# wseaton/gpu-pruner

Hardware: NVIDIA H100
Metric: dcgm_samples_reduced_per_sec (higher is better)
Workload: dtype f32

## Files before the change

### gpu-pruner_b200/csrc/gpr_api.cu

```cuda
#include "../../include/gpr.h"

#include <cuda_runtime.h>
#include <dlfcn.h>
#include <nccl.h>
#include <nvtx3/nvToolsExt.h>

#include <algorithm>
#include <atomic>
#include <chrono>
#include <cmath>
#include <cstdarg>
#include <cstdio>
#include <cstdlib>
#include <cstring>
#include <mutex>
#include <new>
#include <thread>
#include <vector>

#include "gpr_kernels.cuh"
#include "gpr_groups.cuh"
#include "gpr_ring.cuh"
#include "gpr_synth.cuh"
#include "gpr_text_kernels.cuh"

namespace {

using gpr::kLdgUnroll;
using gpr::kLdgWarps;
using gpr::kTmaSmemBudget;
constexpr int kSlots = 256;
constexpr int kMaxChunkEvents = 64;
constexpr int kExchangeDepth = 4;

std::mutex g_err_mu;
char g_create_err[512] = "";

struct NcclApi {
  void* handle = nullptr;
  ncclResult_t (*GetUniqueId)(ncclUniqueId*) = nullptr;
  ncclResult_t (*CommInitRank)(ncclComm_t*, int, ncclUniqueId, int) = nullptr;
  ncclResult_t (*CommDestroy)(ncclComm_t) = nullptr;
  ncclResult_t (*AllGather)(const void*, void*, size_t, ncclDataType_t, ncclComm_t,
                            cudaStream_t) = nullptr;
  const char* (*GetErrorString)(ncclResult_t) = nullptr;
  bool ok = false;
};
NcclApi g_nccl;
std::mutex g_nccl_mu;

bool load_nccl(char* err, size_t n) {
  std::lock_guard<std::mutex> lk(g_nccl_mu);
  if (g_nccl.ok) return true;
  const char* names[] = {"libnccl.so.2", "libnccl.so"};
  for (const char* nm : names) {
    g_nccl.handle = dlopen(nm, RTLD_NOW | RTLD_GLOBAL);
    if (g_nccl.handle) break;
  }
  if (!g_nccl.handle) {
    snprintf(err, n, "NCCL not loadable: %s", dlerror());
    return false;
  }
#define GPR_SYM(field, name)                                              \
  g_nccl.field = reinterpret_cast<decltype(g_nccl.field)>(dlsym(g_nccl.handle, name)); \
  if (!g_nccl.field) {                                                    \
    snprintf(err, n, "NCCL symbol %s missing", name);                     \
    return false;                                                         \
  }
  GPR_SYM(GetUniqueId, "ncclGetUniqueId")
  GPR_SYM(CommInitRank, "ncclCommInitRank")
  GPR_SYM(CommDestroy, "ncclCommDestroy")
  GPR_SYM(AllGather, "ncclAllGather")
  GPR_SYM(GetErrorString, "ncclGetErrorString")
#undef GPR_SYM
  g_nccl.ok = true;
  return true;
}

struct Pending {
  gpr_result* res;
  int slot;
};

}

struct gpr_ctx {
  int device = 0;
  cudaStream_t stream = nullptr;
  bool own_stream = false;
  cudaStream_t copy_stream = nullptr;
  cudaEvent_t ev_k0 = nullptr, ev_k1 = nullptr, ev_t0 = nullptr, ev_t1 = nullptr;
  cudaEvent_t ev_join = nullptr;
  cudaEvent_t ev_chunk[kMaxChunkEvents] = {};
  int sm_count = 0;
  size_t l2_bytes = 0, hbm_bytes = 0;
  int cc_major = 0, cc_minor = 0;
  char name[64] = "";
  int variant = GPR_KERNEL_AUTO;
  int ldg_ctas_per_sm = 2;
  int tma_depth_max = 3;
  int tma_warps = 16;
  int tma_chunk_bytes = 8192;
  size_t chunk_bytes = 32u << 20;
  int parse_ctas_per_sm = 6;

  uint32_t max_pods = 0, max_gpus = 0, max_samples = 0;
  bool cap_power = false;
  float* d_util_stage = nullptr;
  float* d_power_stage = nullptr;
  uint8_t* d_elig_stage = nullptr;
  int64_t* d_created_stage = nullptr;
  size_t gate_cap = 0;

  uint32_t* d_masks[2] = {nullptr, nullptr};
  size_t masks_cap[2] = {0, 0};
  bool masks_dirty = false;
  unsigned int* d_tickets = nullptr;
  unsigned long long* d_acc = nullptr;
  unsigned long long* d_done = nullptr;
  unsigned long long uses[2] = {0, 0};
  unsigned parity = 0;
  bool pdl_enabled = true;
  bool last_was_reduce = false;
  uint32_t* d_bits = nullptr;
  size_t bits_cap = 0;
  uint32_t* d_gather = nullptr;
  size_t gather_cap = 0;
  float* d_smax = nullptr;
  size_t smax_cap = 0;
  uint32_t* d_grouped = nullptr;
  size_t grouped_cap = 0;
  uint32_t* d_gpods = nullptr;
  size_t gpods_cap = 0;
  float* d_gmax = nullptr;
  size_t gmax_cap = 0;
  uint32_t* d_gtable = nullptr;
  size_t gtable_cap = 0;
  uint32_t* d_islots = nullptr;
  size_t islots_cap = 0;
  unsigned int* h_gerr = nullptr;
  unsigned long long* h_counts = nullptr;
  unsigned long long* h_mark = nullptr;
  unsigned int* h_err = nullptr;
  std::vector<Pending> pending;
  std::vector<uint64_t> stamps;
  std::vector<uint64_t> phase_stamps;
  unsigned long long rdv_seq = 0;

  void* d_flush = nullptr;
  size_t flush_bytes = 0;

  float* d_res_util = nullptr;
  float* d_res_power = nullptr;
  uint32_t res_P = 0, res_G = 0, res_T = 0, res_head = 0;
  float* d_idx_util = nullptr;
  float* d_idx_power = nullptr;
  uint32_t idx_ld = 0;
  bool idx_stale = false;
  float* d_cols = nullptr;
  size_t cols_cap = 0;

  uint8_t* d_text[3] = {nullptr, nullptr, nullptr};
  size_t text_cap[3] = {0, 0, 0};
  uint64_t text_n[3] = {0, 0, 0};
  uint64_t* d_marks = nullptr;
  size_t marks_cap = 0;
  unsigned long long* d_mark_counts = nullptr;
  gpr::text::Span* d_spans = nullptr;
  size_t spans_cap = 0;
  float* d_tplane[2] = {nullptr, nullptr};
  size_t tplane_cap[2] = {0, 0};
  static constexpr int kUpThreads = 16, kUpSlots = 2;
  static constexpr size_t kPinnedChunk = 16u << 20;
  static constexpr int kMarkBlocks = 64;
  static constexpr uint32_t kMarkCap = 16384;
  size_t up_chunk = 2u << 20;
  size_t up_slot_bytes = 0;
  unsigned char* h_up_ring = nullptr;
  uint32_t* h_mark_blocks = nullptr;
  uint32_t* d_mark_blocks = nullptr;
  cudaStream_t up_stream[kUpThreads] = {};
  cudaEvent_t up_event[kUpThreads][kUpSlots] = {};
  cudaEvent_t mark_event[kMarkBlocks] = {};
  int up_threads = 8;
  struct ScanPipe* pipe = nullptr;

  ncclComm_t comm = nullptr;
  int rank = 0, world = 1;
  unsigned char* p2p_block = nullptr;
  unsigned char* p2p_peer[gpr::kMaxPeers] = {};
  size_t p2p_gather_off[kExchangeDepth] = {};
  size_t p2p_ll_off[kExchangeDepth] = {};
  bool exchange_ll = true;
  bool exchange_late = false;
  int fold_threads = 256;
  uint32_t p2p_stride = 0;
  bool p2p_ready = false;
  int exchange_debug = 0;
  unsigned int poll_ns = 4000;
  unsigned long long p2p_step = 0;

  uint64_t launches = 0;
  char err[512] = "";
};

void scan_pipe_abort(gpr_ctx* ctx);

namespace {

int fail(gpr_ctx* c, int code, const char* fmt, ...) {
  char buf[512];
  va_list ap;
  va_start(ap, fmt);
  vsnprintf(buf, sizeof buf, fmt, ap);
  va_end(ap);
  if (c) {
    snprintf(c->err, sizeof c->err, "%s", buf);
  } else {
    std::lock_guard<std::mutex> lk(g_err_mu);
    snprintf(g_create_err, sizeof g_create_err, "%s", buf);
  }
  return code;
}

#define CU(call)                                                                          \
  do {                                                                                    \
    cudaError_t e_ = (call);                                                              \
    if (e_ != cudaSuccess)                                                                \
      return fail(ctx, e_ == cudaErrorMemoryAllocation ? GPR_E_NOMEM : GPR_E_CUDA,        \
                  "%s: %s (%s:%d)", #call, cudaGetErrorString(e_), __FILE__, __LINE__);   \
  } while (0)

#define NC(call)                                                                          \
  do {                                                                                    \
    ncclResult_t r_ = (call);                                                             \
    if (r_ != ncclSuccess)                                                                \
      return fail(ctx, GPR_E_NCCL, "%s: %s", #call, g_nccl.GetErrorString(r_));           \
  } while (0)

template <typename T>
int grow(gpr_ctx* ctx, T** p, size_t* cap, size_t need) {
  if (need <= *cap) return GPR_OK;
  if (*p) {
    CU(cudaStreamSynchronize(ctx->stream));
    CU(cudaFree(*p));
    *p = nullptr;
    *cap = 0;
  }
  size_t want = need + need / 4 + 64;
  CU(cudaMalloc(reinterpret_cast<void**>(p), want * sizeof(T)));
  *cap = want;
  return GPR_OK;
}

int env_int(const char* name, int dflt) {
  const char* v = getenv(name);
  return (v && *v) ? atoi(v) : dflt;
}

bool aligned16(const void* p) { return (reinterpret_cast<uintptr_t>(p) & 15u) == 0; }

float threshold_f32(double thr) { return gpr::text::threshold_up(thr); }

bool power_truthy(double thr) { return thr != 0.0 && !std::isnan(thr); }

gpr::LaunchKnobs launch_knobs(const gpr_ctx* ctx) {
  gpr::LaunchKnobs k;
  k.sm_count = ctx->sm_count;
  k.variant = ctx->variant;
  k.ldg_ctas_per_sm = ctx->ldg_ctas_per_sm;
  k.tma_warps = ctx->tma_warps;
  k.tma_chunk_bytes = ctx->tma_chunk_bytes;
  k.tma_depth_max = ctx->tma_depth_max;
  k.fold_threads = ctx->fold_threads;
  return k;
}

template <typename Kernel, typename... Args>
cudaError_t launch_ex(Kernel k, uint32_t grid, uint32_t block, size_t smem, cudaStream_t st, bool pdl,
                      Args... args) {
  cudaLaunchConfig_t cfg = {};
  cfg.gridDim = dim3(grid), cfg.blockDim = dim3(block), cfg.dynamicSmemBytes = smem, cfg.stream = st;
  cudaLaunchAttribute attr[1];
  attr[0].id = cudaLaunchAttributeProgrammaticStreamSerialization;
  attr[0].val.programmaticStreamSerializationAllowed = 1;
  cfg.attrs = attr;
  cfg.numAttrs = pdl ? 1 : 0;
  return cudaLaunchKernelEx(&cfg, k, args...);
}

template <int NW, bool kGroups>
cudaError_t launch_tma(gpr_ctx* ctx, const gpr::ReduceParams& rp, const gpr::ReducePlan& plan, bool pdl) {
  return launch_ex(gpr::k_reduce_tma<NW, kGroups>, plan.grid, plan.block, plan.smem, ctx->stream, pdl, rp, plan.L);
}

template <bool kGroups>
int launch_reduce_as(gpr_ctx* ctx, gpr::ReduceParams& rp, bool tma_ok, bool pdl) {
  if (rp.total_rows == 0) return GPR_OK;
  const gpr::ReducePlan plan = gpr::plan_reduce(launch_knobs(ctx), rp.T, rp.total_rows, tma_ok, rp.util_u8 != 0);
  cudaError_t e;
  if (plan.kernel == gpr::kReduceU8) {
    e = launch_ex(gpr::k_reduce_u8<kLdgWarps, gpr::kU8Unroll, kGroups>, plan.grid, plan.block, 0, ctx->stream, pdl, rp);
  } else if (plan.kernel == gpr::kReduceTma) {
    const int nw = ctx->tma_warps;
    if (nw == 4) e = launch_tma<4, kGroups>(ctx, rp, plan, pdl);
    else if (nw == 16) e = launch_tma<16, kGroups>(ctx, rp, plan, pdl);
    else if (nw == 32) e = launch_tma<32, kGroups>(ctx, rp, plan, pdl);
    else e = launch_tma<8, kGroups>(ctx, rp, plan, pdl);
  } else {
    e = launch_ex(gpr::k_reduce_ldg<kLdgWarps, kLdgUnroll, kGroups>, plan.grid, plan.block, 0, ctx->stream, pdl, rp);
  }
  ctx->launches++;
  CU(e);
  CU(cudaGetLastError());
  return GPR_OK;
}
int launch_reduce(gpr_ctx* ctx, gpr::ReduceParams& rp, bool tma_ok, bool pdl) {
  return rp.grouped ? launch_reduce_as<true>(ctx, rp, tma_ok, pdl) : launch_reduce_as<false>(ctx, rp, tma_ok, pdl);
}

int copy_rows_h2d(gpr_ctx* ctx, void* dst, const void* src, size_t n_rows, uint32_t T,
                  uint64_t ld, size_t esize, cudaStream_t s) {
  if (n_rows == 0) return GPR_OK;
  if (ld == T) {
    CU(cudaMemcpyAsync(dst, src, n_rows * (size_t)T * esize, cudaMemcpyHostToDevice, s));
  } else {
    CU(cudaMemcpy2DAsync(dst, (size_t)T * esize, src, (size_t)ld * esize, (size_t)T * esize, n_rows,
                         cudaMemcpyHostToDevice, s));
  }
  return GPR_OK;
}

struct NvtxRange {
  explicit NvtxRange(const char* name) { nvtxRangePushA(name); }
  ~NvtxRange() { nvtxRangePop(); }
};

int decide_impl(gpr_ctx* ctx, const gpr_window* win, gpr_result* res, bool resident, bool async) {
  if (!ctx) return GPR_E_INVALID;
  NvtxRange nvtx_range(resident ? "gpr_decide_resident" : "gpr_decide");
  if (!win || !res) return fail(ctx, GPR_E_INVALID, "window/result is NULL");
  const size_t win_v1 = offsetof(gpr_window, groups), res_v1 = offsetof(gpr_result, idle_slots);
  if ((win->struct_size != sizeof(gpr_window) && win->struct_size != win_v1) ||
      (res->struct_size != sizeof(gpr_result) && res->struct_size != res_v1))
    return fail(ctx, GPR_E_INVALID, "struct_size mismatch (window %u/%zu or %zu, result %u/%zu or %zu)",
                win->struct_size, sizeof(gpr_window), win_v1, res->struct_size, sizeof(gpr_result), res_v1);
  const uint32_t* const groups = win->struct_size == sizeof(gpr_window) ? win->groups : nullptr;
  uint32_t* const idle_slots = res->struct_size == sizeof(gpr_result) ? res->idle_slots : nullptr;
  CU(cudaSetDevice(ctx->device));

  uint32_t P = win->n_pods, G = win->n_gpus, T = win->n_samples;
  uint64_t ld = win->row_stride ? win->row_stride : T;
  const float* util = win->util;
  const float* power = win->power;
  int in_kind = win->mem_kind;
  const bool u8 = !resident && win->util_format == GPR_FMT_U8B;
  if (!resident && win->util_format != GPR_FMT_F32 && win->util_format != GPR_FMT_U8B)
    return fail(ctx, GPR_E_INVALID, "bad util_format %u", win->util_format);
  if (resident) {
    if (!ctx->d_res_util) return fail(ctx, GPR_E_STATE, "no resident window (gpr_resident_init)");
    P = ctx->res_P, G = ctx->res_G, T = ctx->res_T, ld = T;
    util = ctx->d_res_util;
    power = ctx->d_res_power;
    if (ctx->d_idx_util) {
      if (ctx->idx_stale)
        return fail(ctx, GPR_E_STATE, "the block index is stale: gpr_text_parse(GPR_TEXT_RESIDENT) merged samples "
                    "into the ring; call gpr_resident_reindex before gpr_decide_resident");
      T = ctx->idx_ld, ld = ctx->idx_ld;
      util = ctx->d_idx_util;
      power = ctx->d_idx_power;
    }
  }
  if (in_kind != GPR_MEM_HOST && in_kind != GPR_MEM_DEVICE)
    return fail(ctx, GPR_E_INVALID, "bad mem_kind %d", in_kind);
  if (res->out_mem_kind != GPR_MEM_HOST && res->out_mem_kind != GPR_MEM_DEVICE)
    return fail(ctx, GPR_E_INVALID, "bad out_mem_kind %d", res->out_mem_kind);
  if (G == 0 || T == 0) return fail(ctx, GPR_E_INVALID, "n_gpus and n_samples must be > 0");
  if (G > 256) return fail(ctx, GPR_E_UNSUPPORTED, "n_gpus %u > 256 series slots per pod is not supported", G);
  const uint32_t MW = (G + 31u) / 32u;
  if (ld < T) return fail(ctx, GPR_E_INVALID, "row_stride %llu < n_samples %u",
                          (unsigned long long)ld, T);
  if (P > 0 && !util) return fail(ctx, GPR_E_INVALID, "util is NULL");
  if (!res->decision_bits && P > 0) return fail(ctx, GPR_E_INVALID, "decision_bits is NULL");
  const uint64_t S64 = (uint64_t)P * G;
  if (S64 > 0x7fffffffull) return fail(ctx, GPR_E_INVALID, "too many series (%llu)",
                                       (unsigned long long)S64);
  const uint32_t S = (uint32_t)S64;
  const uint32_t W = (P + 31u) / 32u;
  const bool use_power = power != nullptr && power_truthy(win->power_threshold);
  const bool host_in = !resident && in_kind == GPR_MEM_HOST;
  const bool gates_host = in_kind == GPR_MEM_HOST;
  const bool host_out = res->out_mem_kind == GPR_MEM_HOST;
  const bool fused = ctx->p2p_ready && ctx->world > 1;
  const bool comm = (ctx->comm != nullptr || fused) && ctx->world > 1;
  if (fused && 2u * W > ctx->p2p_stride)
    return fail(ctx, GPR_E_CAPACITY, "n_pods %u exceeds the p2p exchange capacity (%u pods per rank)", P,
                ctx->p2p_stride * 16u);
  if (comm && (P % 32u) != 0)
    return fail(ctx, GPR_E_INVALID, "with a communicator n_pods must be a multiple of 32 (got %u)", P);
  if ((int)ctx->pending.size() >= kSlots)
    return fail(ctx, GPR_E_STATE, "too many outstanding async results; call gpr_sync");
  const bool grouped = groups != nullptr && P > 0;
  if (grouped && in_kind == GPR_MEM_HOST) {
    for (uint32_t p = 0; p < P; ++p) {
      const uint32_t* e = groups + (size_t)p * G;
      for (uint32_t g = 0; g < G; ++g) {
        const uint32_t x = e[g], l = x & gpr::kGroupLeader;
        if ((x & ~(gpr::kGroupLeader | gpr::kGroupUtil)) != 0u || l > g || (e[l] & gpr::kGroupLeader) != l)
          return fail(ctx, GPR_E_INVALID, "gpr_window.groups: malformed entry 0x%x at pod %u slot %u (leader above its "
                      "slot, a leader that does not lead itself, or bits other than 0-7 and GPR_GROUP_UTIL)", x, p, g);
      }
    }
  }

  if (host_in) {
    if ((uint64_t)P * G * T > (uint64_t)ctx->max_pods * ctx->max_gpus * ctx->max_samples)
      return fail(ctx, GPR_E_CAPACITY, "host window %ux%ux%u exceeds the staging capacity of %ux%ux%u cells", P, G, T,
                  ctx->max_pods, ctx->max_gpus, ctx->max_samples);
    if (use_power && !ctx->cap_power)
      return fail(ctx, GPR_E_CAPACITY, "power plane not reserved (GPR_F_POWER_PLANE)");
  }

  int rc;
  const unsigned sset = ctx->parity;
  ctx->parity ^= 1u;
  if (ctx->masks_dirty) {
    CU(cudaMemsetAsync(ctx->d_tickets, 0, 2 * sizeof(unsigned int), ctx->stream));
    CU(cudaMemsetAsync(ctx->d_acc, 0, 6 * sizeof(unsigned long long), ctx->stream));
    ctx->last_was_reduce = false;
  }
  for (int k = 0; k < 2; ++k) {
    const size_t cap_before = ctx->masks_cap[k];
    if ((rc = grow(ctx, &ctx->d_masks[k], &ctx->masks_cap[k], (size_t)2 * P * MW + 16)) != GPR_OK) return rc;
    if (ctx->masks_cap[k] != cap_before || ctx->masks_dirty) {
      CU(cudaMemsetAsync(ctx->d_masks[k], 0, ctx->masks_cap[k] * sizeof(uint32_t), ctx->stream));
      ctx->last_was_reduce = false;
    }
  }
  ctx->masks_dirty = false;
  uint32_t* const masks = ctx->d_masks[sset];
  if ((rc = grow(ctx, &ctx->d_bits, &ctx->bits_cap, (size_t)3 * W + 2)) != GPR_OK) return rc;
  if (comm && !fused &&
      (rc = grow(ctx, &ctx->d_gather, &ctx->gather_cap, (size_t)ctx->world * 2 * W + 2)) != GPR_OK)
    return rc;
  const bool want_smax = res->series_max != nullptr;
  if (want_smax && host_out &&
      (rc = grow(ctx, &ctx->d_smax, &ctx->smax_cap, (size_t)S + 4)) != GPR_OK)
    return rc;
  if (idle_slots && host_out && (rc = grow(ctx, &ctx->d_islots, &ctx->islots_cap, (size_t)P * MW + 4)) != GPR_OK)
    return rc;
  if (grouped) {
    if ((rc = grow(ctx, &ctx->d_grouped, &ctx->grouped_cap, (size_t)P * MW + 4)) != GPR_OK ||
        (rc = grow(ctx, &ctx->d_gpods, &ctx->gpods_cap, (size_t)P + 4)) != GPR_OK ||
        (!want_smax && (rc = grow(ctx, &ctx->d_gmax, &ctx->gmax_cap, (size_t)S + 4)) != GPR_OK) ||
// ... 429 lines not shown
  catch (...) {                                                             \
    return fail(ctxp, GPR_E_INVALID, "unexpected C++ exception");           \
  }

extern "C" {

int gpr_version(void) {
  return GPR_VERSION_MAJOR * 10000 + GPR_VERSION_MINOR * 100 + GPR_VERSION_PATCH;
}

const char* gpr_last_error(const gpr_ctx* ctx) { return ctx ? ctx->err : g_create_err; }

void gpr_destroy(gpr_ctx* ctx) {
  if (!ctx) return;
  cudaSetDevice(ctx->device);
  if (ctx->stream) cudaStreamSynchronize(ctx->stream);
  if (ctx->comm && g_nccl.ok) g_nccl.CommDestroy(ctx->comm);
  for (int r = 0; r < gpr::kMaxPeers; ++r)
    if (ctx->p2p_peer[r] && ctx->p2p_peer[r] != ctx->p2p_block) cudaIpcCloseMemHandle(ctx->p2p_peer[r]);
  if (ctx->p2p_block) cudaFree(ctx->p2p_block);
  void* dev[] = {ctx->d_util_stage, ctx->d_power_stage, ctx->d_elig_stage, ctx->d_created_stage,
                 ctx->d_masks[0],   ctx->d_masks[1],    ctx->d_bits,       ctx->d_gather,
                 ctx->d_smax,       ctx->d_acc,         ctx->d_tickets,    ctx->d_done,
                 ctx->d_flush,      ctx->d_res_util,    ctx->d_res_power,  ctx->d_cols,
                 ctx->d_idx_util,   ctx->d_idx_power,   ctx->d_text[0],    ctx->d_text[1],
                 ctx->d_text[2],    ctx->d_marks,       ctx->d_mark_counts, ctx->d_spans,
                 ctx->d_tplane[0],  ctx->d_tplane[1],  ctx->d_grouped,   ctx->d_gpods,
                 ctx->d_gmax,       ctx->d_gtable,     ctx->d_islots};
  for (void* p : dev)
    if (p) cudaFree(p);
  if (ctx->h_counts) cudaFreeHost(ctx->h_counts);
  scan_pipe_abort(ctx);
  if (ctx->h_up_ring) cudaFreeHost(ctx->h_up_ring);
  if (ctx->h_mark_blocks) cudaFreeHost(ctx->h_mark_blocks);
  if (ctx->d_mark_blocks) cudaFree(ctx->d_mark_blocks);
  for (cudaEvent_t e : ctx->mark_event)
    if (e) cudaEventDestroy(e);
  for (int k = 0; k < gpr_ctx::kUpThreads; ++k) {
    if (ctx->up_stream[k]) cudaStreamDestroy(ctx->up_stream[k]);
    for (cudaEvent_t e : ctx->up_event[k])
      if (e) cudaEventDestroy(e);
  }
  cudaEvent_t evs[] = {ctx->ev_k0, ctx->ev_k1, ctx->ev_t0, ctx->ev_t1, ctx->ev_join};
  for (cudaEvent_t e : evs)
    if (e) cudaEventDestroy(e);
  for (cudaEvent_t e : ctx->ev_chunk)
    if (e) cudaEventDestroy(e);
  if (ctx->copy_stream) cudaStreamDestroy(ctx->copy_stream);
  if (ctx->own_stream && ctx->stream) cudaStreamDestroy(ctx->stream);
  delete ctx;
}

int gpr_create(const gpr_config* cfg, gpr_ctx** out) {
  gpr_ctx* ctx = nullptr;
  GPR_TRY
  if (!cfg || !out) return fail(nullptr, GPR_E_INVALID, "config/out is NULL");
  *out = nullptr;
  if (cfg->struct_size != sizeof(gpr_config))
    return fail(nullptr, GPR_E_INVALID, "gpr_config.struct_size %u != %zu", cfg->struct_size,
                sizeof(gpr_config));
  int n_dev = 0;
  cudaError_t e = cudaGetDeviceCount(&n_dev);
  if (e != cudaSuccess || n_dev == 0)
    return fail(nullptr, GPR_E_CUDA, "no CUDA device (%s); this engine has no CPU fallback",
                e != cudaSuccess ? cudaGetErrorString(e) : "device count 0");
  if (cfg->device < 0 || cfg->device >= n_dev)
    return fail(nullptr, GPR_E_INVALID, "device %d out of range [0,%d)", cfg->device, n_dev);
  gpr_ctx* c = new gpr_ctx();
  c->device = cfg->device;
  auto bail = [&](int code) {
    {
      std::lock_guard<std::mutex> lk(g_err_mu);
      snprintf(g_create_err, sizeof g_create_err, "%s", c->err);
    }
    gpr_destroy(c);
    return code;
  };
  ctx = c;
  auto body = [&]() -> int {
    CU(cudaSetDevice(c->device));
    cudaDeviceProp prop;
    CU(cudaGetDeviceProperties(&prop, c->device));
    c->sm_count = prop.multiProcessorCount;
    c->l2_bytes = (size_t)prop.l2CacheSize;
    c->hbm_bytes = prop.totalGlobalMem;
    c->cc_major = prop.major, c->cc_minor = prop.minor;
    memcpy(c->name, prop.name, sizeof c->name - 1);
    if (prop.major != 9 || prop.minor != 0)
      return fail(c, GPR_E_UNSUPPORTED, "device %s is sm_%d%d; this library is built for sm_90a",
                  prop.name, prop.major, prop.minor);
    if (cfg->stream) {
      c->stream = static_cast<cudaStream_t>(cfg->stream);
    } else {
      CU(cudaStreamCreateWithFlags(&c->stream, cudaStreamNonBlocking));
      c->own_stream = true;
    }
    CU(cudaStreamCreateWithFlags(&c->copy_stream, cudaStreamNonBlocking));
    CU(cudaEventCreate(&c->ev_k0));
    CU(cudaEventCreate(&c->ev_k1));
    CU(cudaEventCreate(&c->ev_t0));
    CU(cudaEventCreate(&c->ev_t1));
    CU(cudaEventCreateWithFlags(&c->ev_join, cudaEventDisableTiming));
    for (cudaEvent_t& ev : c->ev_chunk) CU(cudaEventCreateWithFlags(&ev, cudaEventDisableTiming));
    CU(cudaMalloc(reinterpret_cast<void**>(&c->d_acc), 6 * sizeof(unsigned long long)));
    CU(cudaMalloc(reinterpret_cast<void**>(&c->d_tickets), 2 * sizeof(unsigned int)));
    CU(cudaMalloc(reinterpret_cast<void**>(&c->d_done), 2 * sizeof(unsigned long long)));
    CU(cudaMemset(c->d_acc, 0, 6 * sizeof(unsigned long long)));
    CU(cudaMemset(c->d_tickets, 0, 2 * sizeof(unsigned int)));
    CU(cudaMemset(c->d_done, 0, 2 * sizeof(unsigned long long)));
    c->pdl_enabled = env_int("GPR_PDL", 1) != 0;
    c->up_threads = std::max(1, std::min((int)gpr_ctx::kUpThreads, env_int("GPR_TEXT_UPLOAD_THREADS", 8)));
    c->up_chunk = (size_t)std::max(1, std::min(16, env_int("GPR_TEXT_CHUNK_MB", 2))) << 20;
    c->up_slot_bytes = c->up_chunk + 4096;
    c->exchange_debug = env_int("GPR_DEBUG_EXCHANGE", 0);
    c->poll_ns = (unsigned int)std::max(100, std::min(100000, env_int("GPR_POLL_NS", 4000)));
    if (const char* x = getenv("GPR_EXCHANGE")) {
      c->exchange_ll = strcmp(x, "flags") != 0;
      c->exchange_late = strcmp(x, "pipelined") == 0;
    }
    c->fold_threads = env_int("GPR_FOLD_THREADS", 256);
    if (c->fold_threads != 64 && c->fold_threads != 128 && c->fold_threads != 256) c->fold_threads = 256;
    CU(cudaMallocHost(reinterpret_cast<void**>(&c->h_counts),
                      ((size_t)kSlots * 8 + 2) * sizeof(unsigned long long)));
    memset(c->h_counts, 0, ((size_t)kSlots * 8 + 2) * sizeof(unsigned long long));
    c->h_mark = c->h_counts + (size_t)kSlots * 8;
    c->h_err = reinterpret_cast<unsigned int*>(c->h_mark + 1);
    c->h_gerr = c->h_err + 1;
    c->pending.reserve(kSlots);
    c->stamps.reserve(kSlots);

    c->variant = cfg->kernel_variant;
    if (const char* k = getenv("GPR_KERNEL")) {
      if (!strcmp(k, "ldg")) c->variant = GPR_KERNEL_LDG;
      else if (!strcmp(k, "tma")) c->variant = GPR_KERNEL_TMA;
    }
    if (c->variant < GPR_KERNEL_AUTO || c->variant > GPR_KERNEL_TMA)
      return fail(c, GPR_E_INVALID, "bad kernel_variant %d", c->variant);
    c->ldg_ctas_per_sm = std::max(1, env_int("GPR_LDG_CTAS", 2));
    c->tma_depth_max = std::max(1, env_int("GPR_TMA_DEPTH", 3));
    c->tma_warps = env_int("GPR_TMA_WARPS", 16);
    if (c->tma_warps != 4 && c->tma_warps != 8 && c->tma_warps != 16 && c->tma_warps != 32)
      c->tma_warps = 16;
    c->tma_chunk_bytes = std::min(65536, std::max(512, env_int("GPR_TMA_CHUNK", 8192))) & ~15;
    c->chunk_bytes = (size_t)std::max(1, env_int("GPR_CHUNK_MB", 32)) << 20;
    c->parse_ctas_per_sm = std::max(1, std::min(8, env_int("GPR_PARSE_CTAS", 6)));
    CU(cudaFuncSetAttribute(gpr::k_reduce_tma<4>, cudaFuncAttributeMaxDynamicSharedMemorySize,
                            (int)kTmaSmemBudget));
    CU(cudaFuncSetAttribute(gpr::k_reduce_tma<8>, cudaFuncAttributeMaxDynamicSharedMemorySize,
                            (int)kTmaSmemBudget));
    CU(cudaFuncSetAttribute(gpr::k_reduce_tma<16>, cudaFuncAttributeMaxDynamicSharedMemorySize,
                            (int)kTmaSmemBudget));
    CU(cudaFuncSetAttribute(gpr::k_reduce_tma<32>, cudaFuncAttributeMaxDynamicSharedMemorySize,
                            (int)kTmaSmemBudget));
    CU(cudaFuncSetAttribute(gpr::k_reduce_tma<4, true>, cudaFuncAttributeMaxDynamicSharedMemorySize,
                            (int)kTmaSmemBudget));
    CU(cudaFuncSetAttribute(gpr::k_reduce_tma<8, true>, cudaFuncAttributeMaxDynamicSharedMemorySize,
                            (int)kTmaSmemBudget));
    CU(cudaFuncSetAttribute(gpr::k_reduce_tma<16, true>, cudaFuncAttributeMaxDynamicSharedMemorySize,
                            (int)kTmaSmemBudget));
    CU(cudaFuncSetAttribute(gpr::k_reduce_tma<32, true>, cudaFuncAttributeMaxDynamicSharedMemorySize,
                            (int)kTmaSmemBudget));

    c->max_pods = cfg->max_pods, c->max_gpus = cfg->max_gpus, c->max_samples = cfg->max_samples;
    c->cap_power = (cfg->flags & GPR_F_POWER_PLANE) != 0;
    const size_t cells = (size_t)cfg->max_pods * cfg->max_gpus * cfg->max_samples;
    if (cells) {
      CU(cudaMalloc(reinterpret_cast<void**>(&c->d_util_stage), cells * sizeof(float) + 256));
      if (c->cap_power)
        CU(cudaMalloc(reinterpret_cast<void**>(&c->d_power_stage), cells * sizeof(float) + 256));
    }
    return GPR_OK;
  };
  int rc = body();
  if (rc != GPR_OK) return bail(rc);
  *out = c;
  return GPR_OK;
  GPR_CATCH(nullptr)
}

int gpr_decide_async(gpr_ctx* ctx, const gpr_window* win, gpr_result* res) {
  GPR_TRY
  const int rc = decide_impl(ctx, win, res, false, true);
  if (rc != GPR_OK && ctx) ctx->masks_dirty = true;
  return rc;
  GPR_CATCH(ctx)
}

int gpr_decide_batch_async(gpr_ctx* ctx, const gpr_window* wins, gpr_result* results, uint32_t n) {
  if (!ctx) return GPR_E_INVALID;
  GPR_TRY
  if (n && (!wins || !results)) return fail(ctx, GPR_E_INVALID, "windows/results is NULL");
  for (uint32_t i = 0; i < n; ++i) {
    const int rc = decide_impl(ctx, &wins[i], &results[i], false, true);
    if (rc != GPR_OK) {
      ctx->masks_dirty = true;
      return rc;
    }
  }
  return GPR_OK;
  GPR_CATCH(ctx)
}

int gpr_sync(gpr_ctx* ctx) {
  if (!ctx) return GPR_E_INVALID;
  GPR_TRY
  return sync_impl(ctx);
  GPR_CATCH(ctx)
}

static int decide_blocking(gpr_ctx* ctx, const gpr_window* win, gpr_result* res, bool resident) {
  int rc = decide_impl(ctx, win, res, resident, false);
  if (rc != GPR_OK) {
    if (ctx) {
      cudaStreamSynchronize(ctx->stream);
      ctx->pending.clear();
      ctx->masks_dirty = true;
    }
    return rc;
  }
  rc = sync_impl(ctx);
  if (rc != GPR_OK) return rc;
  float ms = 0.f;
  CU(cudaEventElapsedTime(&ms, ctx->ev_k0, ctx->ev_k1));
  res->kernel_ms = ms;
  return GPR_OK;
}

int gpr_decide(gpr_ctx* ctx, const gpr_window* win, gpr_result* res) {
  GPR_TRY
  return decide_blocking(ctx, win, res, false);
  GPR_CATCH(ctx)
}

int gpr_decide_resident(gpr_ctx* ctx, const gpr_window* win, gpr_result* res) {
  GPR_TRY
  return decide_blocking(ctx, win, res, true);
  GPR_CATCH(ctx)
}

int gpr_resident_init(gpr_ctx* ctx, uint32_t P, uint32_t G, uint32_t T, uint32_t flags) {
  if (!ctx) return GPR_E_INVALID;
  GPR_TRY
  if (P == 0 || G == 0 || T == 0) return fail(ctx, GPR_E_INVALID, "empty resident window");
  if ((uint64_t)P * G > 0x7fffffffull) return fail(ctx, GPR_E_INVALID, "too many series");
  CU(cudaSetDevice(ctx->device));
  CU(cudaStreamSynchronize(ctx->stream));
  if (ctx->d_res_util) CU(cudaFree(ctx->d_res_util));
  if (ctx->d_res_power) CU(cudaFree(ctx->d_res_power));
  ctx->d_res_util = ctx->d_res_power = nullptr;
  const size_t bytes = (size_t)P * G * T * sizeof(float);
  CU(cudaMalloc(reinterpret_cast<void**>(&ctx->d_res_util), bytes));
  CU(cudaMemsetAsync(ctx->d_res_util, 0xFF, bytes, ctx->stream));
  if (flags & GPR_F_POWER_PLANE) {
    CU(cudaMalloc(reinterpret_cast<void**>(&ctx->d_res_power), bytes));
    CU(cudaMemsetAsync(ctx->d_res_power, 0xFF, bytes, ctx->stream));
  }
  if (ctx->d_idx_util) CU(cudaFree(ctx->d_idx_util));
  if (ctx->d_idx_power) CU(cudaFree(ctx->d_idx_power));
  ctx->d_idx_util = ctx->d_idx_power = nullptr, ctx->idx_ld = 0;
  if (flags & GPR_F_BLOCK_INDEX) {
    ctx->idx_ld = gpr::index_ld(T);
    const size_t ib = (size_t)P * G * ctx->idx_ld * sizeof(float);
    CU(cudaMalloc(reinterpret_cast<void**>(&ctx->d_idx_util), ib));
    CU(cudaMemsetAsync(ctx->d_idx_util, 0xFF, ib, ctx->stream));
    if (flags & GPR_F_POWER_PLANE) {
      CU(cudaMalloc(reinterpret_cast<void**>(&ctx->d_idx_power), ib));
      CU(cudaMemsetAsync(ctx->d_idx_power, 0xFF, ib, ctx->stream));
    }
  }
  CU(cudaStreamSynchronize(ctx->stream));
  ctx->res_P = P, ctx->res_G = G, ctx->res_T = T, ctx->res_head = 0;
  ctx->idx_stale = false;
  return GPR_OK;
  GPR_CATCH(ctx)
}

int gpr_resident_reindex(gpr_ctx* ctx) {
  if (!ctx) return GPR_E_INVALID;
  GPR_TRY
  if (!ctx->d_res_util) return fail(ctx, GPR_E_STATE, "no resident window (gpr_resident_init)");
  if (!ctx->d_idx_util) return GPR_OK;
  CU(cudaSetDevice(ctx->device));
  ctx->last_was_reduce = false;
  const size_t rows = (size_t)ctx->res_P * ctx->res_G;
  const uint32_t grid = gpr::ring_grid(rows, ctx->sm_count);
  gpr::k_reindex<<<grid, gpr::kRingThreads, 0, ctx->stream>>>(ctx->d_res_util, (uint32_t)rows, ctx->res_T,
                                                             ctx->d_idx_util, ctx->idx_ld);
  if (ctx->d_res_power)
    gpr::k_reindex<<<grid, gpr::kRingThreads, 0, ctx->stream>>>(ctx->d_res_power, (uint32_t)rows, ctx->res_T,
                                                               ctx->d_idx_power, ctx->idx_ld);
  ctx->launches += ctx->d_res_power ? 2 : 1;
  CU(cudaGetLastError());
  CU(cudaStreamSynchronize(ctx->stream));
  ctx->idx_stale = false;
  return GPR_OK;
  GPR_CATCH(ctx)
}

int gpr_append(gpr_ctx* ctx, const float* util_cols, const float* power_cols, uint32_t n_new,
               uint64_t row_stride, int32_t mem_kind) {
  if (!ctx) return GPR_E_INVALID;
  GPR_TRY
  if (!ctx->d_res_util) return fail(ctx, GPR_E_STATE, "no resident window (gpr_resident_init)");
  if (n_new == 0) return GPR_OK;
  if (!util_cols) return fail(ctx, GPR_E_INVALID, "util_cols is NULL");
  ctx->last_was_reduce = false;
// ... 596 lines not shown
```

### gpu-pruner_b200/csrc/gpr_launch.h

```cpp
#pragma once

#include <stddef.h>
#include <stdint.h>

#include <algorithm>

#include "../../include/gpr.h"

namespace gpr {

constexpr int kLdgWarps = 16;
constexpr int kLdgUnroll = 8;
constexpr int kU8Unroll = 4;
constexpr size_t kTmaSmemBudget = 208 * 1024;
constexpr uint32_t kTmaHeadElems = 128;
constexpr uint32_t kTmaMaxDepth = 32;

#ifndef GPR_TMA_LAYOUT_DEFINED
#define GPR_TMA_LAYOUT_DEFINED
struct TmaLayout {
  uint32_t depth;
  uint32_t stage_bytes;
  uint32_t chunk_elems;
  uint32_t n_chunks;
  uint32_t head_elems;
};
#endif

struct LaunchKnobs {
  int sm_count = 1;
  int variant = GPR_KERNEL_AUTO;
  int ldg_ctas_per_sm = 2;
  int tma_warps = 16;
  int tma_chunk_bytes = 8192;
  int tma_depth_max = 3;
  int fold_threads = 256;
};

enum ReduceKernel { kReduceLdg = 1, kReduceTma = 2, kReduceU8 = 3 };
enum TmaFallback { kNoFallback = 0, kFallbackAlignment = 1, kFallbackSmem = 2 };

struct ReducePlan {
  int kernel;
  int fallback;
  uint32_t grid, block;
  size_t smem;
  TmaLayout L;
};

inline TmaLayout tma_layout(const LaunchKnobs& k, uint32_t T, int nw) {
  TmaLayout L;
  const uint64_t row_bytes = (uint64_t)T * 4u;
  const uint32_t max_chunk = (uint32_t)k.tma_chunk_bytes;
  L.n_chunks = (uint32_t)((row_bytes + max_chunk - 1) / max_chunk);
  uint32_t ce = (T + L.n_chunks - 1) / L.n_chunks;
  ce = (ce + 3u) & ~3u;
  L.chunk_elems = ce;
  L.n_chunks = (T + ce - 1) / ce;
  L.stage_bytes = (ce * 4u + 127u) & ~127u;
  uint32_t d = (uint32_t)((kTmaSmemBudget - 1024) / ((size_t)L.stage_bytes * nw));
  d = std::min<uint32_t>(d, std::min<uint32_t>((uint32_t)k.tma_depth_max, kTmaMaxDepth));
  L.depth = std::max<uint32_t>(d, 1u);
  L.head_elems = std::min<uint32_t>(kTmaHeadElems, ce);
  return L;
}

inline size_t tma_smem_bytes(const TmaLayout& L, int nw) {
  return (size_t)nw * L.depth * L.stage_bytes + (size_t)nw * L.depth * sizeof(uint64_t) + sizeof(uint64_t);
}

inline ReducePlan plan_reduce(const LaunchKnobs& k, uint32_t T, uint32_t total_rows, bool tma_ok, bool util_u8) {
  ReducePlan r = {};
  int variant = k.variant == GPR_KERNEL_AUTO ? GPR_KERNEL_TMA : k.variant;
  if (variant == GPR_KERNEL_TMA && !tma_ok) variant = GPR_KERNEL_LDG, r.fallback = kFallbackAlignment;
  if (variant == GPR_KERNEL_TMA && tma_smem_bytes(tma_layout(k, T, k.tma_warps), k.tma_warps) > kTmaSmemBudget)
    variant = GPR_KERNEL_LDG, r.fallback = kFallbackSmem;
  const uint64_t ldg_need = ((uint64_t)total_rows + kLdgWarps - 1) / kLdgWarps;
  const uint64_t ldg_grid = std::max<uint64_t>(1, std::min<uint64_t>((uint64_t)k.sm_count * k.ldg_ctas_per_sm, ldg_need));
  if (util_u8) {
    r.kernel = kReduceU8, r.fallback = kNoFallback;
    r.grid = (uint32_t)ldg_grid, r.block = kLdgWarps * 32;
  } else if (variant == GPR_KERNEL_TMA) {
    const int nw = k.tma_warps;
    r.kernel = kReduceTma;
    r.grid = (uint32_t)std::max<uint64_t>(1, std::min<uint64_t>((uint64_t)k.sm_count, ((uint64_t)total_rows + nw - 1) / nw));
    r.block = (uint32_t)nw * 32u;
    r.L = tma_layout(k, T, nw);
    r.smem = tma_smem_bytes(r.L, nw);
  } else {
    r.kernel = kReduceLdg;
    r.grid = (uint32_t)ldg_grid, r.block = kLdgWarps * 32;
  }
  return r;
}

inline uint32_t fold_grid(const LaunchKnobs& k, uint32_t P) {
  const uint32_t W = (uint32_t)(((uint64_t)P + 31u) / 32u), warps = (uint32_t)k.fold_threads / 32u;
  return std::max<uint32_t>(1u, std::min<uint32_t>((W + 4u * warps - 1u) / (4u * warps), (uint32_t)k.sm_count));
}

constexpr uint32_t kGroupBlock = 256;
inline uint32_t group_grid(const LaunchKnobs& k, uint32_t P) {
  const uint64_t ctas = ((uint64_t)P + kGroupBlock / 32u - 1u) / (kGroupBlock / 32u);
  return (uint32_t)std::max<uint64_t>(1u, std::min<uint64_t>(ctas, (uint64_t)k.sm_count * 8u));
}

inline uint32_t fold_rounds(const LaunchKnobs& k, uint32_t P) {
  const uint32_t W = (uint32_t)(((uint64_t)P + 31u) / 32u);
  const uint32_t per_round = 4u * fold_grid(k, P) * ((uint32_t)k.fold_threads / 32u);
  return (W + per_round - 1u) / per_round;
}

}
```

Baseline: 1435 billion.

## Add early-exit probe reduction kernel with dynamic row scheduling for ungrouped max

Adds a new TMA-based reduction kernel used by default when no groups or segment max outputs are needed. It loads a small head chunk of each row first, then fetches further chunks only if the running max has not yet settled against the threshold, so it can skip reading the rest of a row. Each warp juggles several rows at once, polling their mbarriers, and pulls new rows from a shared atomic counter. This trades extra per-chunk control flow and smaller TMA transfers for less memory traffic when rows settle early. Results depend on the data, and the new path carries risk around barrier phase handling.

```diff
diff --git a/gpu-pruner_b200/csrc/gpr_api.cu b/gpu-pruner_b200/csrc/gpr_api.cu
--- a/gpu-pruner_b200/csrc/gpr_api.cu
+++ b/gpu-pruner_b200/csrc/gpr_api.cu
@@ -20,6 +20,7 @@
 
 #include "gpr_kernels.cuh"
 #include "gpr_groups.cuh"
+#include "gpr_probe.cuh"
 #include "gpr_ring.cuh"
 #include "gpr_synth.cuh"
 #include "gpr_text_kernels.cuh"
@@ -29,6 +30,7 @@
 using gpr::kLdgUnroll;
 using gpr::kLdgWarps;
 using gpr::kTmaSmemBudget;
+using gpr::kProbeSmemBudget;
 constexpr int kSlots = 256;
 constexpr int kMaxChunkEvents = 64;
 constexpr int kExchangeDepth = 4;
@@ -297,9 +299,13 @@
 template <bool kGroups>
 int launch_reduce_as(gpr_ctx* ctx, gpr::ReduceParams& rp, bool tma_ok, bool pdl) {
   if (rp.total_rows == 0) return GPR_OK;
-  const gpr::ReducePlan plan = gpr::plan_reduce(launch_knobs(ctx), rp.T, rp.total_rows, tma_ok, rp.util_u8 != 0);
+  const bool may_stop = !kGroups && rp.seg[0].smax == nullptr && rp.seg[1].smax == nullptr;
+  const gpr::ReducePlan plan =
+      gpr::plan_reduce(launch_knobs(ctx), rp.T, rp.total_rows, tma_ok, rp.util_u8 != 0, may_stop);
   cudaError_t e;
-  if (plan.kernel == gpr::kReduceU8) {
+  if (plan.kernel == gpr::kReduceProbe) {
+    e = launch_ex(gpr::k_reduce_probe<gpr::kProbeWarps>, plan.grid, plan.block, plan.smem, ctx->stream, pdl, rp, plan.L);
+  } else if (plan.kernel == gpr::kReduceU8) {
     e = launch_ex(gpr::k_reduce_u8<kLdgWarps, gpr::kU8Unroll, kGroups>, plan.grid, plan.block, 0, ctx->stream, pdl, rp);
   } else if (plan.kernel == gpr::kReduceTma) {
     const int nw = ctx->tma_warps;
@@ -1035,6 +1041,8 @@
                             (int)kTmaSmemBudget));
     CU(cudaFuncSetAttribute(gpr::k_reduce_tma<32>, cudaFuncAttributeMaxDynamicSharedMemorySize,
                             (int)kTmaSmemBudget));
+    CU(cudaFuncSetAttribute(gpr::k_reduce_probe<gpr::kProbeWarps>, cudaFuncAttributeMaxDynamicSharedMemorySize,
+                            (int)kProbeSmemBudget));
     CU(cudaFuncSetAttribute(gpr::k_reduce_tma<4, true>, cudaFuncAttributeMaxDynamicSharedMemorySize,
                             (int)kTmaSmemBudget));
     CU(cudaFuncSetAttribute(gpr::k_reduce_tma<8, true>, cudaFuncAttributeMaxDynamicSharedMemorySize,
diff --git a/gpu-pruner_b200/csrc/gpr_launch.h b/gpu-pruner_b200/csrc/gpr_launch.h
--- a/gpu-pruner_b200/csrc/gpr_launch.h
+++ b/gpu-pruner_b200/csrc/gpr_launch.h
@@ -15,6 +15,11 @@
 constexpr size_t kTmaSmemBudget = 208 * 1024;
 constexpr uint32_t kTmaHeadElems = 128;
 constexpr uint32_t kTmaMaxDepth = 32;
+constexpr uint32_t kProbeHeadElems = 32;
+constexpr uint32_t kProbeChunkElems = 512;
+constexpr int kProbeCtasPerSm = 1;
+constexpr int kProbeWarps = 32;
+constexpr size_t kProbeSmemBudget = kTmaSmemBudget;
 
 #ifndef GPR_TMA_LAYOUT_DEFINED
 #define GPR_TMA_LAYOUT_DEFINED
@@ -37,7 +42,7 @@
   int fold_threads = 256;
 };
 
-enum ReduceKernel { kReduceLdg = 1, kReduceTma = 2, kReduceU8 = 3 };
+enum ReduceKernel { kReduceLdg = 1, kReduceTma = 2, kReduceU8 = 3, kReduceProbe = 4 };
 enum TmaFallback { kNoFallback = 0, kFallbackAlignment = 1, kFallbackSmem = 2 };
 
 struct ReducePlan {
@@ -69,8 +74,30 @@
   return (size_t)nw * L.depth * L.stage_bytes + (size_t)nw * L.depth * sizeof(uint64_t) + sizeof(uint64_t);
 }
 
-inline ReducePlan plan_reduce(const LaunchKnobs& k, uint32_t T, uint32_t total_rows, bool tma_ok, bool util_u8) {
+inline TmaLayout probe_layout(uint32_t T, int nw) {
+  TmaLayout L;
+  L.chunk_elems = std::min<uint32_t>(kProbeChunkElems, std::max<uint32_t>((T + 3u) & ~3u, 4u));
+  L.head_elems = std::min<uint32_t>(kProbeHeadElems, L.chunk_elems);
+  L.n_chunks = 1u + (T > L.head_elems ? (T - L.head_elems + L.chunk_elems - 1u) / L.chunk_elems : 0u);
+  L.stage_bytes = (L.chunk_elems * 4u + 127u) & ~127u;
+  const uint32_t d = (uint32_t)((kProbeSmemBudget - 8) / (((size_t)L.stage_bytes + 8) * nw));
+  L.depth = std::max<uint32_t>(std::min<uint32_t>(d, kTmaMaxDepth), 1u);
+  return L;
+}
+
+inline ReducePlan plan_reduce(const LaunchKnobs& k, uint32_t T, uint32_t total_rows, bool tma_ok, bool util_u8,
+                              bool may_stop = false) {
   ReducePlan r = {};
+  if (k.variant == GPR_KERNEL_AUTO && may_stop && tma_ok && !util_u8) {
+    const int nw = kProbeWarps;
+    r.kernel = kReduceProbe;
+    r.grid = (uint32_t)std::max<uint64_t>(
+        1, std::min<uint64_t>((uint64_t)k.sm_count * kProbeCtasPerSm, ((uint64_t)total_rows + nw - 1) / nw));
+    r.block = (uint32_t)nw * 32u;
+    r.L = probe_layout(T, nw);
+    r.smem = tma_smem_bytes(r.L, nw);
+    return r;
+  }
   int variant = k.variant == GPR_KERNEL_AUTO ? GPR_KERNEL_TMA : k.variant;
   if (variant == GPR_KERNEL_TMA && !tma_ok) variant = GPR_KERNEL_LDG, r.fallback = kFallbackAlignment;
   if (variant == GPR_KERNEL_TMA && tma_smem_bytes(tma_layout(k, T, k.tma_warps), k.tma_warps) > kTmaSmemBudget)
diff --git a/gpu-pruner_b200/csrc/gpr_probe.cuh b/gpu-pruner_b200/csrc/gpr_probe.cuh
--- /dev/null
+++ b/gpu-pruner_b200/csrc/gpr_probe.cuh
@@ -0,0 +1,111 @@
+#pragma once
+
+#include "gpr_kernels.cuh"
+
+namespace gpr {
+
+__device__ __forceinline__ bool mbar_test_wait(uint64_t* bar, uint32_t parity) {
+  uint32_t ok;
+  asm volatile(
+      "{\n"
+      ".reg .pred P1;\n"
+      "mbarrier.test_wait.parity.shared::cta.b64 P1, [%1], %2;\n"
+      "selp.u32 %0, 1, 0, P1;\n"
+      "}\n"
+      : "=r"(ok)
+      : "r"(smem_u32(bar)), "r"(parity)
+      : "memory");
+  return ok != 0u;
+}
+
+template <int NW>
+__global__ void __launch_bounds__(NW * 32, kProbeCtasPerSm) k_reduce_probe(ReduceParams p, TmaLayout L) {
+  extern __shared__ __align__(128) unsigned char smem[];
+  const int lane = threadIdx.x & 31;
+  const uint32_t w = threadIdx.x >> 5;
+  const uint32_t D = L.depth;
+  unsigned char* stage0 = smem + (size_t)w * D * L.stage_bytes;
+  uint64_t* const bars = reinterpret_cast<uint64_t*>(smem + (size_t)NW * D * L.stage_bytes);
+  uint64_t* full = bars + w * D;
+  unsigned int* next_row = reinterpret_cast<unsigned int*>(bars + NW * D);
+
+  pdl_launch_dependents();
+  const uint32_t n_rows = cta_row_count(p.total_rows);
+  const uint32_t h = L.head_elems, ce = L.chunk_elems;
+  bool scratch_ok = false;
+
+  if (lane == 0) {
+    for (uint32_t s = 0; s < D; ++s) mbar_init(&full[s], 1);
+    asm volatile("fence.mbarrier_init.release.cluster;" ::: "memory");
+  }
+  if (threadIdx.x == 0) *next_row = NW * D;
+  __syncthreads();
+  const uint64_t pol = l2_evict_first_policy();
+
+  auto issue = [&](uint32_t s, uint32_t j, uint32_t c) {
+    uint32_t seg, local;
+    const float* row = row_ptr(p, blockIdx.x + j * gridDim.x, seg, local);
+    const uint32_t e0 = c ? h + (c - 1u) * ce : 0u;
+    const uint32_t bytes = min(c ? ce : h, p.T - e0) * 4u;
+    if (lane == 0) {
+      mbar_expect_tx(&full[s], bytes);
+      tma_load_1d(stage0 + (size_t)s * L.stage_bytes, row + e0, bytes, &full[s], pol);
+    }
+  };
+  uint32_t my_j = min(w + NW * (uint32_t)lane, n_rows), my_c = 0;
+  float my_m = nan_f();
+  uint32_t live = 0;
+  for (uint32_t s = 0; s < D; ++s) {
+    const uint32_t j = w + NW * s;
+    if (j < n_rows) issue(s, j, 0u), live |= 1u << s;
+  }
+
+  uint32_t phase = 0;
+  while (live) {
+    const bool landed = ((live >> lane) & 1u) && mbar_test_wait(&full[lane], (phase >> lane) & 1u);
+    uint32_t ready = __ballot_sync(0xffffffffu, landed);
+    while (ready) {
+      const uint32_t s = (uint32_t)__ffs(ready) - 1u;
+      ready &= ready - 1u;
+      uint32_t j = __shfl_sync(0xffffffffu, my_j, (int)s);
+      uint32_t c = __shfl_sync(0xffffffffu, my_c, (int)s);
+      float m = __uint_as_float(__shfl_sync(0xffffffffu, __float_as_uint(my_m), (int)s));
+      mbar_wait(&full[s], (phase >> s) & 1u);
+      phase ^= 1u << s;
+      const uint32_t e0 = c ? h + (c - 1u) * ce : 0u;
+      const uint32_t n = min(c ? ce : h, p.T - e0);
+      const float4* v = reinterpret_cast<const float4*>(stage0 + (size_t)s * L.stage_bytes);
+      const uint32_t nv = n >> 2;
+      float m0 = nan_f(), m1 = nan_f();
+      uint32_t k = lane;
+#pragma unroll 2
+      for (; k + 32u < nv; k += 64u) {
+        const float4 a = v[k], b = v[k + 32u];
+        m0 = fold4(m0, a);
+        m1 = fold4(m1, b);
+      }
+      if (k < nv) m0 = fold4(m0, v[k]);
+      m = fmaxf(m, warp_max(fmaxf(m0, m1)));
+      __syncwarp();
+      uint32_t seg, local;
+      (void)row_ptr(p, blockIdx.x + j * gridDim.x, seg, local);
+      const bool is_power = seg ? p.seg[1].is_power != 0 : p.seg[0].is_power != 0;
+      if (e0 + n < p.T && !settles(m, is_power, p.thr)) {
+        issue(s, j, ++c);
+      } else {
+        uint32_t next = 0;
+        if (lane == 0) {
+          if (!scratch_ok) wait_scratch_free(p), scratch_ok = true;
+          publish_row(p, seg, local, m, false);
+          next = atomicAdd(next_row, 1u);
+        }
+        j = min(__shfl_sync(0xffffffffu, next, 0), n_rows), c = 0, m = nan_f();
+        if (j < n_rows) issue(s, j, 0u);
+        else live &= ~(1u << s);
+      }
+      if ((uint32_t)lane == s) my_j = j, my_c = c, my_m = m;
+    }
+  }
+}
+
+}
diff --git a/profiles/h100_probe/short_runs.py b/profiles/h100_probe/short_runs.py
--- /dev/null
+++ b/profiles/h100_probe/short_runs.py
@@ -0,0 +1,31 @@
+import sys, os
+sys.path.insert(0, os.getcwd())
+import numpy as np, torch
+import gpu_pruner_b200 as g
+P, G, T, SEED, ROT = 10000, 4, 1800, 0x5EED0002, 4
+eng = g.IdleEngine(device=0)
+wins = []
+for i in range(ROT):
+    u = torch.full((P, G, T), float("nan"), dtype=torch.float32, device="cuda:0")
+    e = torch.zeros(P, dtype=torch.uint8, device="cuda:0")
+    torch.cuda.synchronize()
+    eng.synth_fill(SEED + 16 * i, 0, u, 0, P, G, T)
+    eng.synth_eligible(SEED + 16 * i, e, 0, P)
+    wins.append((u, e))
+db = torch.zeros((P + 31) // 32, dtype=torch.int32, device="cuda:0")
+torch.cuda.synchronize()
+step = lambda i, b=False: eng.decide_ptr(wins[i % ROT][0], P, G, T, db, eligible=wins[i % ROT][1], blocking=b)
+batch = eng.make_batch([dict(util=wins[i % ROT][0], eligible=wins[i % ROT][1], P=P, G=G, T=T, decision_bits=db)
+                        for i in range(200)])
+for i in range(20): step(i)
+eng.sync()
+out = []
+for K in (5, 20, 200):
+    best = []
+    for rep in range(7):
+        eng.timer_begin(); eng.decide_batch_async(batch, K); ms = eng.timer_end(); eng.sync()
+        best.append(ms / K * 1e3)
+    out.append(f"K={K}: min {min(best):.2f} med {sorted(best)[3]:.2f}")
+iso = sorted(step(i, True).kernel_ms for i in range(21))
+out.append(f"iso med {iso[10]*1e3:.2f} min {iso[0]*1e3:.2f}")
+print(sys.argv[1] if len(sys.argv) > 1 else "", " | ".join(out), flush=True)
```

New measurement: 1595 billion, median of 6. 1.11x the previous value.
